# matheusfalcaopinto/triple-hybrid-rag

Measured on AMD Instinct MI355X. Metric: queries/sec (fused top-10), higher is better.
Workload: dtype f16 MFMA shortlist scan (f32 accumulate) + f64 rescoring of the f32 rows; 1 GPU; 1000000-doc / 768-d dense-only brute-force cosine top-10 (BASELINE.json configs[1]); pipeline=dense, docs=1000000, dim=768, semantic_top_k=100, fused_top_k=10, shortlist=f16, parallelism=single GPU, world_size_seen=1, rescued_queries=0

## Files before the change

triple-hybrid-rag_amd/csrc/dense.hip:

```cpp
#include <stdlib.h>

#include "dense_common.hpp"

namespace thr {

constexpr double QREG_AIM_1M = 1448.0;
constexpr int QREG_KS = 32;
struct DenseKnobs {
    bool forced_q;
    int shape;
    bool forced32;
    double aim_1m;
    int ks;
};
static const DenseKnobs& dense_knobs() {
    static const DenseKnobs knobs = [] {
        DenseKnobs K;
        const char* e = getenv("THR_DENSE_F16");
        K.forced_q = e && e[0] == 'q';
        e = getenv("THR_DENSE_MFMA");
        K.shape = (e && atoi(e) == 32) ? 32 : 16;
        e = getenv("THR_DENSE_QW");
        K.forced32 = e && atoi(e) == 32;
        e = getenv("THR_DENSE_AIM");
// ... 39 lines not shown
    p.ntiles = (n_queries + p.qtile - 1) / p.qtile;
    p.qpad = p.ntiles * p.qtile;
    const int64_t groups = (n_docs + MF_ROWS - 1) / MF_ROWS;
    p.sampled = n_docs > CAND_CAP / 2;
    const int ks_cap = p.packed ? dense_knobs().ks : 64;
    p.ksample = kprime < ks_cap ? kprime : ks_cap;
    double aim = (p.packed ? dense_knobs().aim_1m : 4096.0) * sqrt((double)n_docs / 1.0e6);
    const double aim_lo = 8.0 * kprime < 4096.0 ? 8.0 * kprime : 4096.0;
    aim = aim < aim_lo ? aim_lo : aim > 4096.0 ? 4096.0 : aim;
    int64_t target = (int64_t)((double)n_docs * (double)p.ksample / aim);
    if (target > SAMPLE_MAX) target = SAMPLE_MAX;
    if (target < 4 * (int64_t)p.ksample) target = 4 * (int64_t)p.ksample;
    int64_t sg = (target + MF_ROWS - 1) / MF_ROWS;
    if (sg > groups) sg = groups;
    p.sample_stride = sg > 0 ? groups / sg : 1;
    if (p.sample_stride < 1) p.sample_stride = 1;
    p.sample_groups = p.sampled ? sg : 0;
    p.sample_docs = p.sample_groups * MF_ROWS;
    p.groups = groups;
    p.tile_cap = p.packed ? 1 : p.qtile * (CAND_CAP / 2);
    const size_t qpad = (size_t)p.qpad;
    Arena A{(char*)ws};
    p.tau = A.take<float>(qpad);
    p.qerr = A.take<float>(qpad);
    if (kind != KIND_F16) p.qerr = nullptr;
    p.cnt = A.take<int>(qpad * (p.packed ? QREG_MAX_SEG : 1));
    p.tcnt = A.take<int>(p.ntiles);
    p.cand = A.take<Cand>(qpad * CAND_CAP);
    p.tlist = A.take<Cand>((size_t)p.ntiles * p.tile_cap);
    p.sample = A.take<float>(p.packed ? qpad * (size_t)QREG_MAX_SEG * SAMPLE_TOP : qpad * (size_t)p.sample_docs);
    p.qfrag = A.take<_Float16>(p.packed ? qpad * (size_t)dim : 0);
    p.sel_rows = A.take<int32_t>(qpad * SEL_BIG_BAND);
    p.sel_meta = A.take<int32_t>(4 * qpad);
    p.total = A.total;
    return p;
}

dim3 scan_grid(int ntiles, int64_t n_row_tiles, int waves, bool* shared_rows, int blocks_per_cu,
               int m_cap) {
    const int cus = num_cus() * blocks_per_cu;
    int64_t m_max = n_row_tiles / (8 * (int64_t)waves);
    if (m_max < 1) m_max = 1;
    if (m_max > m_cap) m_max = m_cap;
    int best_m = 1;
    double best_eff = 0.0;
    for (int m = 1; m <= (int)m_max; ++m) {
        const int64_t g = 8 * (int64_t)m * ntiles;
        const int64_t rounds = (g + cus - 1) / cus;
        const double eff = (double)g / (double)(rounds * cus);
        if (eff > best_eff + 1e-9) {
            best_eff = eff;
            best_m = m;
        }
    }
    *shared_rows = ntiles > 1;
    return dim3((unsigned)(8 * best_m * ntiles), 1u);
}

bool scan_nt(bool shared_rows) { return !shared_rows; }


template <int MODE>
static int launch_scan(const DensePlan& P, const DenseIndex& X, const DenseBatch& B, int* nseg = nullptr) {
    constexpr bool all = MODE == MODE_ALL;
    const int64_t units = all ? P.sample_groups : P.groups, stride = all ? P.sample_stride : 1;
    const float* tau = all ? nullptr : P.tau;
    float* smp = all ? P.sample : nullptr;
    const int64_t ld = all ? P.sample_docs : 0;
    if (P.packed)
        return launch_scan_f16q<MODE>(X.dim, X.docs16, P.qfrag, P.ntiles, units, stride, tau,
                                      all ? nullptr : P.cnt, all ? nullptr : P.cand, smp, B.st,
                                      nseg, X.doc_coll, B.query_coll, B.n_queries);
    const int32_t* doc_coll = all ? nullptr : X.doc_coll;
    const int32_t* query_coll = all ? nullptr : B.query_coll;
    int* tcnt = all ? nullptr : P.tcnt;
    Cand* tlist = all ? nullptr : P.tlist;
    const int tile_cap = all ? 0 : P.tile_cap;
    if (P.anydim)
        return launch_scan_anydim<MODE>(X.dim, X.docs, X.inv_norm, X.n_docs, B.queries, B.n_queries, P.ntiles,
                                        units, stride, tau, tcnt, tlist, tile_cap, smp, ld, B.st, doc_coll,
                                        query_coll);
    if (P.kind == KIND_F16)
        return launch_scan_f16<MODE>(X.dim, P.nq, X.docs, X.inv_norm, X.n_docs, B.queries, B.n_queries,
                                     P.ntiles, units, stride, tau, tcnt, tlist, tile_cap, smp, ld, B.st,
                                     doc_coll, query_coll);
    return launch_scan_mfma<MODE>(X.dim, X.docs, X.inv_norm, X.n_docs, B.queries, B.n_queries, P.ntiles,
                                  units, stride, tau, tcnt, tlist, tile_cap, smp, ld, B.st, doc_coll,
                                  query_coll);
}

static int dense_pipeline(const DensePlan& P, const DenseIndex& X, const DenseBatch& B,
                          const DensePhase& S) {
    int rc, nseg = 0, sample_nseg = 0;
    if (S.phase != PIPE_FINISH) {
        if (!P.packed) {
            hipError_t e = hipMemsetAsync(P.cnt, 0, (char*)P.cand - (char*)P.cnt, B.st);
            if (e != hipSuccess) return (int)e;
        }
        if (P.packed && (rc = launch_pack_queries(X.dim, B.queries, B.n_queries, P.qpad, P.qfrag, P.qerr, B.st)))
            return rc;
        if (P.sampled && (rc = launch_scan<MODE_ALL>(P, X, B, &sample_nseg))) return rc;
        if ((rc = launch_threshold(P, X, B, P.packed ? sample_nseg : 0))) return rc;
        if ((rc = launch_scan<MODE_FILTER>(P, X, B, &nseg))) return rc;
        if (!P.packed && (rc = launch_bucket(P, B.st))) return rc;
    } else if (P.packed) {
        if ((rc = launch_scan_f16q<MODE_FILTER, true>(X.dim, X.docs16, P.qfrag, P.ntiles, P.groups, 1,
                                                      nullptr, nullptr, nullptr, nullptr, B.st, &nseg)))
            return rc;
    }
    if ((rc = launch_band(P, X, B, S, nseg))) return rc;
    if (S.phase == PIPE_SHORTLIST) return THR_OK;
    return launch_rescore(P, X, B);
}

}

using namespace thr;

extern "C" size_t thr_dense_workspace_bytes(int64_t n_docs, int dim, int n_queries, int kprime) {
    if (n_docs <= 0 || n_queries <= 0) return 0;
    return make_plan(nullptr, n_docs, n_queries, kprime, KIND_F32, dim, false).total;
}

static int dense_args_ok(const void* docs, const void* dnorm, const void* inv_norm,
                         const void* queries, const void* a, const void* b, const void* c,
                         const void* d, const void* ws, int64_t n_docs, int n_queries, int k,
                         int kprime) {
    THR_RETURN_IF(!docs || !dnorm || !inv_norm || !queries || !a || !b || !c || !d || !ws,
                  THR_ERR_INVALID);
    THR_RETURN_IF(n_docs <= 0 || n_queries <= 0 || k <= 0 || kprime < k ||
                      kprime > THR_DENSE_MAX_K,
                  THR_ERR_INVALID);
// ... 209 lines not shown
```

triple-hybrid-rag_amd/csrc/dense_common.hpp:

```cpp
#pragma once
#include <type_traits>

#include "thr_common.hpp"

namespace thr {

constexpr int CHUNK = 256;
constexpr int MODE_ALL = 0, MODE_FILTER = 1;
constexpr int CAND_CAP = 16384;
constexpr int SAMPLE_MAX = 1 << 20;
constexpr int WBUF = 256;
constexpr int ROW_BITS = 27;
constexpr uint32_t ROW_MASK = (1u << ROW_BITS) - 1;
constexpr int ROW_BITS_F16 = 25;
constexpr int SEL_BIG_BAND = 1024;
constexpr int QREG_MAX_SEG = 1024;
constexpr int SAMPLE_TOP = 4;
constexpr int CS_BINS = 4096;

struct Cand {
    float score;
    uint32_t doc;
};

// ... 49 lines not shown
           (sizeof(Cand) * WBUF + sizeof(float4) * MF2_STAGE_F4) * H_WAVES;
}
inline int f16_pick_nq(int dim) { return f16_lds_bytes(dim, 2) <= 160 * 1024 ? 2 : 1; }

inline bool anydim_ok(int dim) {
    return dim >= THR_DENSE_ANYDIM_STEP && dim <= THR_DENSE_ANYDIM_MAX && dim % THR_DENSE_ANYDIM_STEP == 0;
}
inline int anydim_qt(int dim) { return dim <= 768 ? 64 : dim <= 1536 ? 32 : 16; }
inline size_t anydim_lds_bytes(int dim) {
    return sizeof(_Float16) * (size_t)anydim_qt(dim) * (size_t)dim + sizeof(Cand) * WBUF * H_WAVES;
}

inline bool f16_tiles_agree() {
    for (int dim : {512, 768, 1024})
        if (anydim_qt(dim) != 32 * f16_pick_nq(dim)) return false;
    return true;
}

inline double scan_eps(int dim) {
    const double u = 5.9604644775390625e-08;
    return ((double)dim + 16.0) * u;
}

constexpr int KIND_F32 = 0, KIND_F16 = 1;
struct DensePlan {
    int kind;
    bool anydim;
    bool packed;
    int nq, qtile, ntiles, qpad, row_bits, ksample, tile_cap;
    bool sampled;
    int64_t groups, sample_groups, sample_stride, sample_docs;
    float* tau;
    float* qerr;
    int* cnt;
    int* tcnt;
    Cand *cand, *tlist;
    float* sample;
    _Float16* qfrag;
    int32_t *sel_rows, *sel_meta;
    size_t total;
};
struct DenseIndex {
    const float *docs, *inv_norm;
    int64_t n_docs;
    int dim;
    const double* dnorm = nullptr;
    int64_t id_base = 0;
    const int32_t* doc_coll = nullptr;
    const _Float16* docs16 = nullptr;
    double doc_rel_err = 0.0;
};
struct DenseBatch {
    const float* queries;
    int n_queries, k, kprime;
    const int32_t* query_coll;
    hipStream_t st;
    double* out_scores = nullptr;
    int64_t* out_ids = nullptr;
    int32_t* out_counts = nullptr;
    uint32_t* out_flags = nullptr;
};
enum { PIPE_ALL = 0, PIPE_SHORTLIST = 1, PIPE_FINISH = 2 };
struct DensePhase {
    int phase = PIPE_ALL;
    float* top_lb = nullptr;
    int top_m = 0;
// ... 7 lines not shown
int qreg_shape(int dim);
int qreg_qw(int dim);
int qreg_max_queries(int dim);
dim3 scan_grid(int ntiles, int64_t n_row_tiles, int waves, bool* shared_rows, int blocks_per_cu = 1,
               int m_cap = 64);
bool scan_nt(bool shared_rows);

template <int MODE>
int launch_scan_mfma(int dim, const float* docs, const float* inv_norm, int64_t n_docs,
                     const float* queries, int n_queries, int ntiles, int64_t n_row_tiles,
                     int64_t tile_stride, const float* tau, int* tile_cnt, Cand* tile_list,
                     int tile_cap, float* sample, int64_t sample_ld, hipStream_t st,
                     const int32_t* doc_coll = nullptr, const int32_t* query_coll = nullptr);
template <int MODE>
int launch_scan_f16(int dim, int nq, const float* rows32, const float* inv_norm, int64_t n_docs,
                    const float* queries, int n_queries, int ntiles, int64_t n_row_tiles,
                    int64_t tile_stride, const float* tau, int* tile_cnt, Cand* tile_list,
                    int tile_cap, float* sample, int64_t sample_ld, hipStream_t st,
                    const int32_t* doc_coll = nullptr, const int32_t* query_coll = nullptr);
template <int MODE>
int launch_scan_anydim(int dim, const float* rows32, const float* inv_norm, int64_t n_docs,
                       const float* queries, int n_queries, int ntiles, int64_t n_row_tiles,
                       int64_t tile_stride, const float* tau, int* tile_cnt, Cand* tile_list,
                       int tile_cap, float* sample, int64_t sample_ld, hipStream_t st,
                       const int32_t* doc_coll = nullptr, const int32_t* query_coll = nullptr);
template <int MODE, bool PROF = false>
int launch_scan_f16q(int dim, const _Float16* rows16, const _Float16* qfrag, int n_qtiles,
                     int64_t n_row_tiles, int64_t tile_stride, const float* tau, int* seg_cnt,
                     Cand* cand, float* sample, hipStream_t st,
                     int* nseg_out = nullptr, const int32_t* doc_coll = nullptr,
                     const int32_t* query_coll = nullptr, int n_queries = 1 << 30,
                     unsigned long long* stamps = nullptr, int* n_blocks = nullptr);
int launch_pack_queries(int dim, const float* queries, int n_queries, int qpad, _Float16* qfrag,
                        float* qerr, hipStream_t st);
int launch_quantize_f16(const float* docs, int64_t n_docs, int dim, _Float16* docs16,
                        unsigned int* max_rel_err, hipStream_t st);
int launch_threshold(const DensePlan& P, const DenseIndex& X, const DenseBatch& B, int sample_nseg);
int launch_bucket(const DensePlan& P, hipStream_t st);
int launch_band(const DensePlan& P, const DenseIndex& X, const DenseBatch& B, const DensePhase& S, int nseg);
int launch_rescore(const DensePlan& P, const DenseIndex& X, const DenseBatch& B);
int launch_merge_scoped(const double* slab_s, const int64_t* slab_id, int n_queries, int n_slabs, int k,
                        int64_t id_base, const int32_t* query_scope, int n_scopes, double* out_scores,
                        int64_t* out_ids, int32_t* out_counts, uint32_t* out_flags, hipStream_t st);

}
```

triple-hybrid-rag_amd/csrc/dense_rescore.hip:

```cpp
#include "dense_common.hpp"

namespace thr {

constexpr int RS_STRIDE = 9;
constexpr int RR_WAVES = 2, RR_THREADS = 64 * RR_WAVES, RR_ROWS = 64;
static size_t rescore_lds_bytes(int dim) {
    return sizeof(double) * dim + sizeof(float4) * RR_WAVES * RR_ROWS * RS_STRIDE;
}
template <int U, bool TAIL = false>
__device__ __forceinline__ double rescore_pass(const f32x4* (&rp)[8], f32x4* stage, const double* q64,
                                               int nchunk, int lane, int lrow, int lch) {
    constexpr int D = U >= 2 ? 16 / U : 8;
    f32x4 nxt[D][U];
#pragma unroll
    for (int dd = 0; dd < D; ++dd)
#pragma unroll
        for (int u = 0; u < U; ++u) nxt[dd][u] = rp[u][8 * (TAIL && dd >= nchunk ? nchunk - 1 : dd)];
    double dot = 0.0;
#pragma unroll 1
    for (int ck0 = 0; ck0 < nchunk; ck0 += D) {
#pragma unroll
        for (int dd = 0; dd < D; ++dd) {
            const int ck = ck0 + dd;
            if (TAIL && ck >= nchunk) break;
// ... 84 lines not shown
        double sim = -INFINITY;
        if (dn > 0.0) sim = qn > 0.0 ? __ddiv_rn(dot, __dmul_rn(qn, dn)) : 0.0;
        s_s[p] = sim;
        s_id[p] = sim == -INFINITY ? INT64_MAX : row + id_base;
    }
    __syncthreads();
    for (int p = threadIdx.x; p < ns; p += RR_THREADS) {
        const double ms = s_s[p];
        const int64_t mi = s_id[p];
        if (mi == INT64_MAX) continue;
        int rank = 0;
        for (int i = 0; i < ns; ++i) rank += better(s_s[i], s_id[i], ms, mi) ? 1 : 0;
        o_s[rank] = ms;
        o_id[rank] = mi;
    }
    __syncthreads();

    int mine_valid = 0;
    for (int i = threadIdx.x; i < k; i += RR_THREADS) {
        const bool ok = o_s[i] > -INFINITY;
        mine_valid += ok ? 1 : 0;
        out_scores[(int64_t)q * k + i] = ok ? o_s[i] : -INFINITY;
        out_ids[(int64_t)q * k + i] = ok ? o_id[i] : -1;
    }
    if (mine_valid) atomicAdd(&n_valid, mine_valid);
    __syncthreads();
    if (threadIdx.x == 0) {
        const int valid = n_valid;
        uint32_t flag = overflow ? THR_FLAG_OVERFLOW : 0u;
        bool cert;
        if (overflow) {
            cert = false;
        } else if (floor32 == -INFINITY) {
            cert = true;
        } else {
            const float gF = __uint_as_float((uint32_t)sel_meta[4 * q + 3]);
            const bool own = valid >= k && s_qn > 0.0 && (o_s[k - 1] - (double)floor32 / s_qn) > eps;
            const bool all = gF > -INFINITY && s_qn > 0.0 &&
                             ((double)gF / s_qn - (double)floor32 / s_qn) > eps;
            cert = own || all;
        }
        out_flags[q] = flag | (cert ? THR_FLAG_CERTIFIED : 0u);
        out_counts[q] = valid;
    }
}

int launch_rescore(const DensePlan& P, const DenseIndex& X, const DenseBatch& B) {
    const bool tail = X.dim % 256 != 0, big_lds = X.dim > 1024;
    for (auto kern : {tail ? rescore_rank<THR_DENSE_MAX_K, true> : rescore_rank<THR_DENSE_MAX_K, false>,
                      tail ? rescore_rank<SEL_BIG_BAND, true> : rescore_rank<SEL_BIG_BAND, false>}) {
        int rc;
        if (big_lds) {
            rc = launch_lds(kern, dim3(B.n_queries), dim3(RR_THREADS), rescore_lds_bytes(X.dim), B.st,
                            X.docs, X.dnorm, X.dim, X.id_base, B.queries, B.k, scan_eps(X.dim),
                            X.doc_rel_err, (const float*)P.qerr, (const int32_t*)P.sel_rows,
                            (const int32_t*)P.sel_meta, B.out_scores, B.out_ids, B.out_counts, B.out_flags);
        } else {
            hipLaunchKernelGGL(kern, dim3(B.n_queries), dim3(RR_THREADS), rescore_lds_bytes(X.dim), B.st,
                               X.docs, X.dnorm, X.dim, X.id_base, B.queries, B.k, scan_eps(X.dim),
                               X.doc_rel_err, P.qerr, P.sel_rows, P.sel_meta, B.out_scores, B.out_ids,
                               B.out_counts, B.out_flags);
            rc = launch_status();
        }
        if (rc) return rc;
    }
    return THR_OK;
}
// ... 3 lines not shown
```

triple-hybrid-rag_amd/csrc/dense_scan_f16q.hip:

```cpp
#include "dense_scan_f16q.hpp"

namespace thr {

template <int MODE, bool PROF>
int launch_scan_f16q(int dim, const _Float16* rows16, const _Float16* qfrag, int n_qtiles,
                            int64_t n_row_tiles, int64_t tile_stride, const float* tau, int* seg_cnt,
                            Cand* cand, float* sample, hipStream_t st,
                            int* nseg_out, const int32_t* doc_coll,
                            const int32_t* query_coll, int n_queries,
                            unsigned long long* stamps, int* n_blocks) {
    bool shared_rows = false;
    const bool stag = qreg_staggered(dim);
    const dim3 grid = scan_grid(n_qtiles, n_row_tiles, 1, &shared_rows, (!stag && dim <= 768) ? 2 : 1, 32);
    const int shape = qreg_shape(dim);
    const int nseg = (shape == 16 ? 4 : 2) * (int)(grid.x / n_qtiles);
    if (nseg_out) *nseg_out = nseg;
    if (n_blocks) *n_blocks = (int)grid.x;
    if (PROF && !stamps) return THR_OK;
#define THR_QS_LAUNCH(DIM, SHAPE)                                                                 \
    return launch_lds(dense_scan_f16qs<DIM, MODE, SHAPE>, grid, dim3(QS_NW * 64),                 \
                      QStag<DIM>::LDS_BYTES, st, (const f32x4*)rows16, (const f32x4*)qfrag,       \
                      n_qtiles, n_row_tiles, tile_stride, tau, seg_cnt, cand, CAND_CAP / nseg,    \
                      sample, doc_coll, query_coll, n_queries);
    if (stag) {
        if (dim == 512 && shape == 32) THR_QS_LAUNCH(512, 32)
        if (dim == 512) THR_QS_LAUNCH(512, 16)
        if (shape == 32) THR_QS_LAUNCH(768, 32)
        THR_QS_LAUNCH(768, 16)
    }
#undef THR_QS_LAUNCH
#define THR_Q_LAUNCH(DIM, SHAPE)                                                                  \
    return launch_lds(dense_scan_f16q<DIM, MODE, PROF, SHAPE>, grid, dim3(Q_NW * 64),             \
                      QScan<DIM>::LDS_BYTES, st, (const f32x4*)rows16, (const f32x4*)qfrag,       \
                      n_qtiles, n_row_tiles, tile_stride, tau, seg_cnt, cand, CAND_CAP / nseg,    \
                      sample, doc_coll, query_coll, n_queries, stamps);
    switch (dim) {
        case 512: if (shape == 16) THR_Q_LAUNCH(512, 16) THR_Q_LAUNCH(512, 32)
        case 768: if (shape == 16) THR_Q_LAUNCH(768, 16) THR_Q_LAUNCH(768, 32)
        case 1024:
            if (shape == 16 && qreg_qw(dim) == 48) THR_Q_LAUNCH(1024, 48)
            if (shape == 16) THR_Q_LAUNCH(1024, 16)
            THR_Q_LAUNCH(1024, 32)
        default: return THR_ERR_UNSUPPORTED;
    }
#undef THR_Q_LAUNCH
}

int launch_pack_queries(int dim, const float* queries, int n_queries, int qpad,
                               _Float16* qfrag, float* qerr, hipStream_t st) {
    const dim3 grid((unsigned)(qpad / 32));
    const bool s16 = qreg_shape(dim) == 16;
#define THR_PACK(DIM, SHAPE) \
    hipLaunchKernelGGL((pack_queries_f16<DIM, SHAPE>), grid, dim3(256), 0, st, queries, n_queries, (f32x4*)qfrag, qerr)
    switch (dim) {
        case 512: if (s16) THR_PACK(512, 16); else THR_PACK(512, 32); break;
        case 768: if (s16) THR_PACK(768, 16); else THR_PACK(768, 32); break;
        case 1024: if (s16) THR_PACK(1024, 16); else THR_PACK(1024, 32); break;
        default: return THR_ERR_UNSUPPORTED;
    }
#undef THR_PACK
    return launch_status();
}

int launch_quantize_f16(const float* docs, int64_t n_docs, int dim, _Float16* docs16,
                        unsigned int* max_rel_err, hipStream_t st) {
    if (docs16) {
        THR_RETURN_IF(dim % 16 != 0, THR_ERR_UNSUPPORTED);
        const int64_t n_pad = (n_docs + 31) / 32 * 32;
        hipLaunchKernelGGL(quantize_f16_norm, dim3((unsigned)((n_pad + 3) / 4)), dim3(256), 0, st,
                           docs, n_docs, dim, qreg_shape(dim), docs16, max_rel_err);
        return launch_status();
    }
    hipLaunchKernelGGL(measure_f16_error, dim3((unsigned)((n_docs + 3) / 4)), dim3(256), 0, st, docs,
                       n_docs, dim, max_rel_err);
    return launch_status();
}

#define THR_INSTANTIATE(MODE, PROF)                                                                    \
    template int launch_scan_f16q<MODE, PROF>(int, const _Float16*, const _Float16*, int, int64_t, int64_t, \
                                              const float*, int*, Cand*, float*, hipStream_t, int*, \
                                              const int32_t*, const int32_t*, int, unsigned long long*, int*);
THR_INSTANTIATE(MODE_ALL, false)
THR_INSTANTIATE(MODE_FILTER, false)
THR_INSTANTIATE(MODE_FILTER, true)
#undef THR_INSTANTIATE

// ... 2 lines not shown
```

triple-hybrid-rag_amd/csrc/dense_scan_f16q.hpp:

```cpp
#pragma once
#include "dense_common.hpp"

namespace thr {

constexpr int Q_RING = 4;
constexpr int Q_NW = 4;

template <int DIM>
struct QScan {
    static constexpr int KS = DIM / 16;
    static constexpr int HS = KS / 2;
    static constexpr int HALF_BYTES = HS * 1024;
    static constexpr int PER_CU = DIM <= 768 ? 2 : 1;
    static constexpr int NB = (160 * 1024 / PER_CU) / HALF_BYTES > 4 ? 4 : (160 * 1024 / PER_CU) / HALF_BYTES;
    static constexpr int PER = HS / Q_NW;
#ifndef THR_Q_RING_1024
#define THR_Q_RING_1024 8
#endif
    static constexpr int RING = PER_CU == 1 ? THR_Q_RING_1024 : Q_RING;
#ifdef Q_PROBE_EXTRA
    static constexpr int VM_PER_PIECE = 2, LDS_BYTES = NB * HALF_BYTES + 32 * 1024;
#else
    static constexpr int VM_PER_PIECE = 1, LDS_BYTES = NB * HALF_BYTES;
#endif
    static_assert(HS % Q_NW == 0 && NB >= 3, "half tile must split evenly over the waves; >= 3 buffers");
};

template <int DIM, int SHAPE>
__global__ __launch_bounds__(256) void pack_queries_f16(const float* __restrict__ queries,
                                                        int n_queries, f32x4* __restrict__ qfrag,
                                                        float* __restrict__ qerr) {
    constexpr int KS = DIM / 16;
    const int lane = threadIdx.x & 63, wave = threadIdx.x >> 6;
    __shared__ double red[4][4][32];
    double e = 0.0, nn = 0.0, e_hi = 0.0, n_hi = 0.0;
#pragma unroll 4
    for (int s = wave; s < KS; s += 4) {
        int q, d0;
        if constexpr (SHAPE == 32) {
            q = blockIdx.x * 32 + (lane & 31);
            d0 = 16 * s + 8 * (lane >> 5);
        } else {
            q = blockIdx.x * 32 + 16 * (s / (KS / 2)) + (lane & 15);
            d0 = 32 * (s % (KS / 2)) + 8 * (lane >> 4);
        }
        f32x4 lo = {0.f, 0.f, 0.f, 0.f}, hi = lo;
        if (q < n_queries) {
            const f32x4* src = reinterpret_cast<const f32x4*>(queries + (int64_t)q * DIM + d0);
            lo = src[0];
            hi = src[1];
        }
        const f32x4 packed = pack_f16x8(lo, hi);
        qfrag[((int64_t)blockIdx.x * KS + s) * 64 + lane] = packed;
        const half8 hv = __builtin_bit_cast(half8, packed);
        double e1 = 0.0, n1 = 0.0;
#pragma unroll
        for (int j = 0; j < 8; ++j) {
            const float v = j < 4 ? lo[j] : hi[j - 4];
            const double d = (double)v - (double)(float)hv[j];
            e1 += d * d;
            n1 += (double)v * (double)v;
        }
        if (SHAPE == 32 || s < KS / 2) {
            e += e1;
            nn += n1;
        } else {
            e_hi += e1;
            n_hi += n1;
        }
    }
    if constexpr (SHAPE == 32) {
        e += __shfl_xor(e, 32, WAVE);
        nn += __shfl_xor(nn, 32, WAVE);
        if (lane < 32) {
            red[wave][0][lane] = e;
            red[wave][1][lane] = nn;
        }
    } else {
#pragma unroll
        for (int m = 16; m <= 32; m <<= 1) {
            e += __shfl_xor(e, m, WAVE);
            nn += __shfl_xor(nn, m, WAVE);
            e_hi += __shfl_xor(e_hi, m, WAVE);
            n_hi += __shfl_xor(n_hi, m, WAVE);
        }
        if (lane < 16) {
            red[wave][0][lane] = e;
            red[wave][1][lane] = nn;
            red[wave][0][16 + lane] = e_hi;
            red[wave][1][16 + lane] = n_hi;
        }
    }
    __syncthreads();
    if (threadIdx.x < 32) {
        double es = 0.0, ns = 0.0;
#pragma unroll
        for (int w = 0; w < 4; ++w) {
            es += red[w][0][threadIdx.x];
            ns += red[w][1][threadIdx.x];
        }
        const float rel = ns > 0.0 ? (float)sqrt(es / ns) : 0.f;
        qerr[blockIdx.x * 32 + threadIdx.x] = __uint_as_float(__float_as_uint(rel) + 1u);
    }
}

#define QS_RD(dst, ks) \
    asm volatile("ds_read_b128 %0, %1 offset:%2" : "=v"(dst) : "v"(abase), "n"((ks) * 1024) : "memory")
template <int S, int HS, int RING>
__device__ __forceinline__ void qs_fill(f32x4 (&a)[RING], uint32_t abase) {
    if constexpr (S < RING && S < HS) {
        QS_RD(a[S], S);
        qs_fill<S + 1, HS>(a, abase);
    }
}
template <int SHAPE>
struct QAcc;
template <>
struct QAcc<32> {
    static constexpr int NQL = 1, SEGS = 2;
    static constexpr int QW = 32, NQB = 2, NREG = 16;
    f32x16 v;
    __device__ __forceinline__ void zero() {
#pragma unroll
        for (int x = 0; x < 16; ++x) v[x] = 0.f;
    }
    template <int X> __device__ __forceinline__ float get() const { return v[X]; }
    template <int X> static __device__ __forceinline__ int row(int lane) { return (X & 3) + 8 * (X >> 2) + 4 * (lane >> 5); }
    template <int X> static constexpr int qsel() { return 0; }
    static __device__ __forceinline__ int query(int lane, int) { return lane & 31; }
    static __device__ __forceinline__ int seg(int lane) { return lane >> 5; }
};
template <>
struct QAcc<48> {
    static constexpr int NQL = 3, SEGS = 4;
    static constexpr int QW = 48, NQB = 3, NREG = 24;
// ... 70 lines not shown
            if (qc[qs] != -1 && doc_coll[row] != qc[qs]) return;
            if (slot[qs] < end[qs]) {
                const uint64_t word = (uint64_t)__float_as_uint(v) | ((uint64_t)row << 32);
                asm volatile("global_store_dwordx2 %0, %1, %2" ::"v"(slot[qs]), "v"(word), "s"(cand) : "memory");
            }
            slot[qs] += 8;
        }
    }
    template <int X>
    __device__ __forceinline__ void all(const QAcc<SHAPE>& acc, uint32_t row0, int lane) {
        if constexpr (X < QAcc<SHAPE>::NREG) {
            one<X>(acc, row0, lane);
            all<X + 1>(acc, row0, lane);
        }
    }
};

template <int SHAPE>
struct QTop {
    static constexpr int NQL = QAcc<SHAPE>::NQL;
    const int32_t* doc_coll;
    int qc[NQL];
    float t[NQL][SAMPLE_TOP];
    __device__ __forceinline__ void init() {
#pragma unroll
        for (int u = 0; u < NQL; ++u)
#pragma unroll
            for (int j = 0; j < SAMPLE_TOP; ++j) t[u][j] = -INFINITY;
    }
    template <int X>
    __device__ __forceinline__ void one(const QAcc<SHAPE>& acc, uint32_t row0, int lane) {
        constexpr int qs = QAcc<SHAPE>::template qsel<X>();
        float x = acc.template get<X>();
        x = x == x ? x : -INFINITY;
        if (doc_coll && qc[qs] != -1 && x > -INFINITY) {
            const uint32_t row = row0 + (uint32_t)QAcc<SHAPE>::template row<X>(lane);
            if (doc_coll[row] != qc[qs]) x = -INFINITY;
        }
#pragma unroll
        for (int j = 0; j < SAMPLE_TOP; ++j) {
            const float hi = fmaxf(t[qs][j], x);
            x = fminf(t[qs][j], x);
            t[qs][j] = hi;
        }
    }
    template <int X>
    __device__ __forceinline__ void all(const QAcc<SHAPE>& acc, uint32_t row0, int lane) {
        if constexpr (X < QAcc<SHAPE>::NREG) {
            one<X>(acc, row0, lane);
            all<X + 1>(acc, row0, lane);
        }
    }
    __device__ __forceinline__ void store(float* __restrict__ sample, int u, int64_t q, int nseg, int seg) const {
        float* dst = sample + (q * nseg + seg) * SAMPLE_TOP;
#pragma unroll
        for (int j = 0; j < SAMPLE_TOP; ++j) dst[j] = t[u][j];
    }
};

template <int S, int HS, int K0, int KS, int PER, int SHAPE, int HF, int RING, int NBQ, typename Issue>
__device__ __forceinline__ void qsx_steps_pe(f32x4 (&a)[RING], const f32x4 (&bq)[NBQ], QAcc<SHAPE>& acc,
                                             uint32_t abase, Issue& issue_piece, QEmit<SHAPE>& em,
                                             const QAcc<SHAPE>& prv, uint32_t row_prv, int lane) {
    if constexpr (S < HS) {
        constexpr int left = HS - S - 1 < RING - 1 ? HS - S - 1 : RING - 1;
        asm volatile("s_waitcnt lgkmcnt(%1)" : "+v"(a[S % RING]) : "n"(left) : "memory");
        qsx_mfma<S, K0, KS, SHAPE>(a[S % RING], bq, acc);
        if constexpr (S + RING < HS) QS_RD(a[S % RING], S + RING);
        constexpr int every = HS / PER;
        if constexpr (S % every == 1 && S / every < PER) issue_piece(std::integral_constant<int, S / every>{});
        constexpr int NRH = QAcc<SHAPE>::NREG / 2, j = S * NRH / HS;
        if constexpr ((S + 1) * NRH / HS > j) em.template one<NRH * HF + j>(prv, row_prv, lane);
        qsx_steps_pe<S + 1, HS, K0, KS, PER, SHAPE, HF, RING, NBQ>(a, bq, acc, abase, issue_piece, em, prv, row_prv, lane);
    }
}
#undef QS_RD

// ... 484 lines not shown
```

triple-hybrid-rag_amd/csrc/dense_select.hip:

```cpp
#include "dense_common.hpp"

namespace thr {

constexpr int BUCKET_BLOCKS = 32;
__global__ __launch_bounds__(256) void bucket_candidates(const int* __restrict__ tile_cnt,
                                                         const Cand* __restrict__ tile_list,
                                                         int tile_cap, int qtile, int row_bits,
                                                         int* __restrict__ cand_cnt,
                                                         Cand* __restrict__ cand) {
    __shared__ int count[128], base[128], fill[128];
    const uint32_t row_mask = (1u << row_bits) - 1u;
    const int tile = blockIdx.y;
    int n = tile_cnt[tile];
    n = n < tile_cap ? n : tile_cap;
    const int per = (n + gridDim.x - 1) / gridDim.x;
    const int lo = blockIdx.x * per, hi = lo + per < n ? lo + per : n;
    const Cand* list = tile_list + (int64_t)tile * tile_cap;
    if (threadIdx.x < 128) count[threadIdx.x] = fill[threadIdx.x] = 0;
    __syncthreads();
    for (int i = lo + threadIdx.x; i < hi; i += blockDim.x)
        atomicAdd(&count[list[i].doc >> row_bits], 1);
    __syncthreads();
    if (threadIdx.x < qtile && count[threadIdx.x] > 0)
        base[threadIdx.x] = atomicAdd(&cand_cnt[tile * qtile + threadIdx.x], count[threadIdx.x]);
// ... 196 lines not shown
    sweep([&](float v) { m = fmaxf(m, v); });
#pragma unroll
    for (int o = 32; o > 0; o >>= 1) m = fmaxf(m, __shfl_xor(m, o, WAVE));
    if (lane == 0) kred[wave] = m;
    if (threadIdx.x == 0) kcnt = 0;
    for (int i = threadIdx.x; i < CS_BINS; i += 256) hist[i] = 0;
    __syncthreads();
    m = fmaxf(fmaxf(kred[0], kred[1]), fmaxf(kred[2], kred[3]));
    if (m > 0.f && m < INFINITY) {
        const float thr = 0.5f * m, scale = 4095.f / (m - thr);
        int c = 0;
        sweep([&](float v) {
            if (v >= thr) {
                const int bn = (int)((v - thr) * scale);
                atomicAdd(&hist[bn > CS_BINS - 1 ? CS_BINS - 1 : bn], 1);
                ++c;
            }
        });
#pragma unroll
        for (int o = 32; o > 0; o >>= 1) c += __shfl_xor(c, o, WAVE);
        if (lane == 0 && c) atomicAdd(&kcnt, c);
        __syncthreads();
        if (kcnt >= kk) {
            coarse_find_bin(hist, kk, aux);
            if (threadIdx.x == 0) tau[q] = thr + (float)aux[0] / scale;
            return;
        }
        __syncthreads();
    }
    const uint32_t key = block_coarse_select([&](int i) { return fkey(val(i)); }, n_sample, kk, hist, aux);
    if (threadIdx.x == 0) tau[q] = coarse_value(key);
}

constexpr int KT_REG = 16;
static_assert(QREG_MAX_SEG * SAMPLE_TOP <= 256 * KT_REG, "kth_select_top holds every kept value in registers");
__global__ __launch_bounds__(256) void kth_select_top(const float* __restrict__ sample, int n_vals, int kk,
                                                      const float* __restrict__ queries, int n_queries,
                                                      int dim, float* __restrict__ tau) {
    __shared__ int hist[256];
    __shared__ int wsum[4];
    __shared__ int bc[2];
    __shared__ int flag;
    const int q = blockIdx.x, t = threadIdx.x, lane = t & 63, wave = t >> 6;
    if (query_is_void(queries, n_queries, dim, q, &flag)) {
        if (t == 0) tau[q] = INFINITY;
        return;
    }
    if (n_vals < kk) {
        if (t == 0) tau[q] = -INFINITY;
        return;
    }
    uint32_t key[KT_REG];
#pragma unroll
    for (int u = 0; u < KT_REG; ++u) {
        const int i = t + u * 256;
        key[u] = fkey(i < n_vals ? sample[(int64_t)q * n_vals + i] : -INFINITY);
    }
    uint32_t prefix = 0, mask = 0;
    int remaining = kk;
#pragma unroll 1
    for (int shift = 24; shift >= 0; shift -= 8) {
        hist[t] = 0;
        __syncthreads();
#pragma unroll
        for (int u = 0; u < KT_REG; ++u)
            if (t + u * 256 < n_vals && (key[u] & mask) == prefix) atomicAdd(&hist[(key[u] >> shift) & 255], 1);
        __syncthreads();
        const int mine = hist[255 - t];
        int incl = mine;
#pragma unroll
        for (int o = 1; o < 64; o <<= 1) {
            const int v = __shfl_up(incl, o, WAVE);
            if (lane >= o) incl += v;
        }
        if (lane == 63) wsum[wave] = incl;
        __syncthreads();
        for (int x = 0; x < wave; ++x) incl += wsum[x];
        if (incl - mine < remaining && remaining <= incl) {
            bc[0] = 255 - t;
            bc[1] = incl - mine;
        }
        __syncthreads();
        remaining -= bc[1];
        prefix |= (uint32_t)bc[0] << shift;
        mask |= 255u << shift;
    }
    if (t == 0) tau[q] = fkey_inv(prefix);
}

constexpr int SEL_THREADS = 256;
constexpr int SEL_REG = 16;
constexpr int SEL_FLAT = 8192;
static size_t band_lds_bytes(int dim) { return sizeof(float) * dim + sizeof(int) * CS_BINS; }
constexpr int CAPB = SEL_BIG_BAND;
template <bool TOPM>
__global__ __launch_bounds__(SEL_THREADS, 4) void select_band(
    int dim, const float* __restrict__ queries, const float* __restrict__ tau,
    const int* __restrict__ cand_cnt, const Cand* __restrict__ cand,
    const int* __restrict__ tile_cnt, int tile_cap, int qtile, int k, int kprime, double eps32,
    double doc_relerr, const float* __restrict__ qerr, int nseg, int seg_cap,
    const int32_t* __restrict__ doc_coll, const int32_t* __restrict__ query_coll,
    int32_t* __restrict__ sel_rows, int32_t* __restrict__ sel_meta,
    const float* __restrict__ gfloor, const float* __restrict__ lb_all, int n_shards, int lb_m,
    float* __restrict__ top_lb, int top_m) {
    extern __shared__ float4 lds_sel[];
    __shared__ int aux[8];
    __shared__ int bc[4];
    __shared__ int32_t s_id[CAPB];
    __shared__ int n_sel;
    __shared__ double wsum[4];
    float* lds_qv = reinterpret_cast<float*>(lds_sel);
    int* hist = reinterpret_cast<int*>(lds_sel + dim / 4);

    const int q = blockIdx.x;
    const int lane = threadIdx.x & 63, wave = threadIdx.x >> 6;
    const double eq = qerr ? (double)qerr[q] : 0.0;
    const double eps = eps32 + doc_relerr * (1.0 + eq) + eq;
    const Cand* c = cand + (int64_t)q * CAND_CAP;
    const Cand* my_ptr = c + threadIdx.x;
    int my_n, my_c[4] = {0, 0, 0, 0};
    bool overflow, flat = true;
    int n;
    __shared__ unsigned short src_off[SEL_FLAT];
    if (nseg == 0) {
        const int cnt = cand_cnt[q];
        overflow = cnt > CAND_CAP || tile_cnt[q / qtile] > tile_cap;
        n = cnt < CAND_CAP ? cnt : CAND_CAP;
        my_n = n > (int)threadIdx.x ? (n - (int)threadIdx.x + SEL_THREADS - 1) / SEL_THREADS : 0;
    } else {
        __shared__ int wtot[4];
        bool over = false;
        int tot = 0;
#pragma unroll
        for (int x = 0; x < 4; ++x) {
            const int sg = (int)threadIdx.x + x * SEL_THREADS;
            int sc = sg < nseg ? cand_cnt[(int64_t)q * nseg + sg] : 0;
            over |= sc > seg_cap;
// ... 31 lines not shown
        int sg = threadIdx.x;
#pragma unroll
        for (int x = 0; x < 3; ++x)
            if (u >= my_c[x]) {
                u -= my_c[x];
                sg += SEL_THREADS;
            } else {
                break;
            }
        return c[(int64_t)sg * seg_cap + u];
    };

    const int qc = query_coll ? query_coll[q] : -1;
    auto load_cand = [&](int u) -> Cand {
        Cand e = cand_at(u);
        if (qc != -1 && doc_coll[e.doc] != qc) e.score = -INFINITY;
        return e;
    };
    Cand mine[SEL_REG];
#pragma unroll
    for (int u = 0; u < SEL_REG; ++u) mine[u] = u < my_n ? load_cand(u) : Cand{-INFINITY, 0u};
    if (qc != -1) {
        __shared__ int n_pass;
        if (threadIdx.x == 0) n_pass = 0;
        __syncthreads();
        int mine_ok = 0;
#pragma unroll
        for (int u = 0; u < SEL_REG; ++u) mine_ok += (u < my_n && mine[u].score > -INFINITY) ? 1 : 0;
        for (int u = SEL_REG; u < my_n; ++u) mine_ok += load_cand(u).score > -INFINITY ? 1 : 0;
        if (mine_ok) atomicAdd(&n_pass, mine_ok);
        __syncthreads();
        n = n_pass;
    }
    for (int i = threadIdx.x; i < dim / 4; i += SEL_THREADS)
        lds_sel[i] = reinterpret_cast<const float4*>(queries + (int64_t)q * dim)[i];
    if (threadIdx.x == 0) n_sel = 0;
    __syncthreads();

    {
        double part = 0.0;
        for (int i = threadIdx.x; i < dim; i += SEL_THREADS) part += (double)lds_qv[i] * (double)lds_qv[i];
        for (int o = 32; o > 0; o >>= 1) part += __shfl_xor(part, o, WAVE);
        if (lane == 0) wsum[wave] = part;
        __syncthreads();
    }
    const double qn_hi = sqrt(wsum[0] + wsum[1] + wsum[2] + wsum[3]) * (1.0 + 1e-6);

    float gF = -INFINITY;
    if (!TOPM) {
        if (gfloor) {
            gF = gfloor[q];
        } else if (lb_all && n_shards * lb_m >= k) {
            __shared__ float s_gF;
            float* fv = reinterpret_cast<float*>(hist);
            const int nv = n_shards * lb_m, nv4 = (nv + 3) & ~3;
            for (int i = threadIdx.x; i < nv4; i += SEL_THREADS)
                fv[i] = i < nv ? lb_all[((int64_t)(i / lb_m) * gridDim.x + q) * lb_m + i % lb_m] : -INFINITY;
            if (threadIdx.x == 0) s_gF = -INFINITY;
            __syncthreads();
            const f32x4* fv4 = reinterpret_cast<const f32x4*>(fv);
            for (int i = threadIdx.x; i < nv; i += SEL_THREADS) {
                const float v = fv[i];
                if (!(v > -INFINITY)) continue;
                int rank = 0;
#pragma unroll 4
                for (int j = 0; j < nv4; j += 4) {
                    const f32x4 w = fv4[j >> 2];
                    rank += (w.x > v || (w.x == v && j < i)) ? 1 : 0;
                    rank += (w.y > v || (w.y == v && j + 1 < i)) ? 1 : 0;
                    rank += (w.z > v || (w.z == v && j + 2 < i)) ? 1 : 0;
                    rank += (w.w > v || (w.w == v && j + 3 < i)) ? 1 : 0;
                }
                if (rank == k - 1) s_gF = v;
            }
            __syncthreads();
            gF = s_gF;
            __syncthreads();
        }
    }
// ... 175 lines not shown
    for (int i = threadIdx.x; i < ns; i += SEL_THREADS) sel_rows[(int64_t)q * CAPB + i] = s_id[i];
    if (threadIdx.x == 0) {
        sel_meta[4 * q + 0] = ns;
        sel_meta[4 * q + 1] = (int32_t)__float_as_uint(floor32);
        sel_meta[4 * q + 2] = overflow ? 1 : 0;
        sel_meta[4 * q + 3] = (int32_t)__float_as_uint(gF);
    }
}

__global__ __launch_bounds__(256) void dense_floor_kernel(const float* __restrict__ lb, int n_shards,
                                                          int n_queries, int m, int k,
                                                          float* __restrict__ gfloor) {
    extern __shared__ float fl_v[];
    const int q = blockIdx.x, n = n_shards * m;
    for (int i = threadIdx.x; i < n; i += blockDim.x)
        fl_v[i] = lb[((int64_t)(i / m) * n_queries + q) * m + i % m];
    if (threadIdx.x == 0) gfloor[q] = -INFINITY;
    __syncthreads();
    if (n < k) return;
    for (int i = threadIdx.x; i < n; i += blockDim.x) {
        const float v = fl_v[i];
        if (!(v > -INFINITY)) continue;
        int rank = 0;
        for (int j = 0; j < n; ++j) {
            const float w = fl_v[j];
            rank += (w > v || (w == v && j < i)) ? 1 : 0;
        }
        if (rank == k - 1) gfloor[q] = v;
    }
}

int launch_threshold(const DensePlan& P, const DenseIndex& X, const DenseBatch& B, int sample_nseg) {
    if (P.sampled && sample_nseg > 0) {
        hipLaunchKernelGGL(kth_select_top, dim3(P.qpad), dim3(256), 0, B.st, (const float*)P.sample,
                           sample_nseg * SAMPLE_TOP, P.ksample, B.queries, B.n_queries, X.dim, P.tau);
        return launch_status();
    }
    hipLaunchKernelGGL(kth_select, dim3(P.qpad), dim3(256), 0, B.st,
                       P.sampled ? (const float*)P.sample : nullptr, P.sample_docs, (int)P.sample_docs,
                       P.ksample, B.queries, B.n_queries, X.dim, P.tau, P.packed ? nullptr : P.qerr,
                       X.doc_coll, B.query_coll, MF_ROWS, P.sampled ? P.sample_stride : (int64_t)1,
                       X.n_docs);
    return launch_status();
}

int launch_bucket(const DensePlan& P, hipStream_t st) {
    hipLaunchKernelGGL(bucket_candidates, dim3(BUCKET_BLOCKS, P.ntiles), dim3(256), 0, st, P.tcnt,
                       P.tlist, P.tile_cap, P.qtile, P.row_bits, P.cnt, P.cand);
    return launch_status();
}

int launch_band(const DensePlan& P, const DenseIndex& X, const DenseBatch& B, const DensePhase& S,
                int nseg) {
    const bool topm = S.phase == PIPE_SHORTLIST;
    hipLaunchKernelGGL(topm ? select_band<true> : select_band<false>, dim3(B.n_queries),
                       dim3(SEL_THREADS), band_lds_bytes(X.dim), B.st, X.dim, B.queries, P.tau, P.cnt,
                       P.cand, P.tcnt, P.tile_cap, P.qtile, B.k, B.kprime, scan_eps(X.dim),
                       X.doc_rel_err, P.qerr, nseg, nseg ? CAND_CAP / nseg : 0, X.doc_coll,
                       B.query_coll, P.sel_rows, P.sel_meta, S.gfloor, S.lb_all, S.n_shards,
                       topm ? 0 : S.top_m, S.top_lb, topm ? S.top_m : 0);
    return launch_status();
}

}

using namespace thr;

extern "C" int thr_dense_floor(const float* top_lb, int n_shards, int n_queries, int m, int k,
                               float* gfloor, thr_stream_t stream) {
    clear_status();
    THR_RETURN_IF(!top_lb || !gfloor || n_shards <= 0 || n_queries <= 0 || m <= 0 || k <= 0, THR_ERR_INVALID);
    THR_RETURN_IF((int64_t)n_shards * m > 8192, THR_ERR_CAPACITY);
    hipLaunchKernelGGL(dense_floor_kernel, dim3(n_queries), dim3(256), sizeof(float) * n_shards * m,
                       (hipStream_t)stream, top_lb, n_shards, n_queries, m, k, gfloor);
    return launch_status();
}
```

Measured before the change: 756,100 queries/s.

## Precompute query norms and void flags in pack kernel; wave-level kth select

The query-packing kernel now also writes each query's f64 norm bound and an all-zero flag. The select_band kernel can then skip reloading the query and re-reducing its norm, and the threshold kernel no longer rescans the query to detect void queries. kth_select_top is rewritten to process one query per wave with a bitwise ballot radix select, replacing the block-wide shared-memory histogram passes. The sampled top-4 insertion uses fmed3 instead of a max/min chain, and the NaN guard moves from the scan to a NaN check on the norm in the rescore certification. The change adds workspace buffers and shifts NaN handling semantics.

Result: no change. 760,600 queries/s (median of 6 runs) (+0.6%).

```diff
diff --git a/triple-hybrid-rag_amd/csrc/dense.hip b/triple-hybrid-rag_amd/csrc/dense.hip
--- a/triple-hybrid-rag_amd/csrc/dense.hip
+++ b/triple-hybrid-rag_amd/csrc/dense.hip
@@ -95,6 +95,8 @@
     p.qfrag = A.take<_Float16>(p.packed ? qpad * (size_t)dim : 0);
     p.sel_rows = A.take<int32_t>(qpad * SEL_BIG_BAND);
     p.sel_meta = A.take<int32_t>(4 * qpad);
+    p.qn_hi = p.packed ? A.take<double>(qpad) : nullptr;
+    p.qvoid = p.packed ? A.take<int>(qpad) : nullptr;
     p.total = A.total;
     return p;
 }
@@ -160,7 +162,7 @@
             hipError_t e = hipMemsetAsync(P.cnt, 0, (char*)P.cand - (char*)P.cnt, B.st);
             if (e != hipSuccess) return (int)e;
         }
-        if (P.packed && (rc = launch_pack_queries(X.dim, B.queries, B.n_queries, P.qpad, P.qfrag, P.qerr, B.st)))
+        if (P.packed && (rc = launch_pack_queries(X.dim, B.queries, B.n_queries, P.qpad, P.qfrag, P.qerr, P.qn_hi, P.qvoid, B.st)))
             return rc;
         if (P.sampled && (rc = launch_scan<MODE_ALL>(P, X, B, &sample_nseg))) return rc;
         if ((rc = launch_threshold(P, X, B, P.packed ? sample_nseg : 0))) return rc;
diff --git a/triple-hybrid-rag_amd/csrc/dense_common.hpp b/triple-hybrid-rag_amd/csrc/dense_common.hpp
--- a/triple-hybrid-rag_amd/csrc/dense_common.hpp
+++ b/triple-hybrid-rag_amd/csrc/dense_common.hpp
@@ -105,6 +105,8 @@
     int64_t groups, sample_groups, sample_stride, sample_docs;
     float* tau;
     float* qerr;
+    double* qn_hi;
+    int* qvoid;
     int* cnt;
     int* tcnt;
     Cand *cand, *tlist;
@@ -178,7 +180,7 @@
                      const int32_t* query_coll = nullptr, int n_queries = 1 << 30,
                      unsigned long long* stamps = nullptr, int* n_blocks = nullptr);
 int launch_pack_queries(int dim, const float* queries, int n_queries, int qpad, _Float16* qfrag,
-                        float* qerr, hipStream_t st);
+                        float* qerr, double* qn_hi, int* qvoid, hipStream_t st);
 int launch_quantize_f16(const float* docs, int64_t n_docs, int dim, _Float16* docs16,
                         unsigned int* max_rel_err, hipStream_t st);
 int launch_threshold(const DensePlan& P, const DenseIndex& X, const DenseBatch& B, int sample_nseg);
diff --git a/triple-hybrid-rag_amd/csrc/dense_rescore.hip b/triple-hybrid-rag_amd/csrc/dense_rescore.hip
--- a/triple-hybrid-rag_amd/csrc/dense_rescore.hip
+++ b/triple-hybrid-rag_amd/csrc/dense_rescore.hip
@@ -140,7 +140,7 @@
         if (overflow) {
             cert = false;
         } else if (floor32 == -INFINITY) {
-            cert = true;
+            cert = s_qn == s_qn;
         } else {
             const float gF = __uint_as_float((uint32_t)sel_meta[4 * q + 3]);
             const bool own = valid >= k && s_qn > 0.0 && (o_s[k - 1] - (double)floor32 / s_qn) > eps;
diff --git a/triple-hybrid-rag_amd/csrc/dense_scan_f16q.hip b/triple-hybrid-rag_amd/csrc/dense_scan_f16q.hip
--- a/triple-hybrid-rag_amd/csrc/dense_scan_f16q.hip
+++ b/triple-hybrid-rag_amd/csrc/dense_scan_f16q.hip
@@ -47,11 +47,11 @@
 }
 
 int launch_pack_queries(int dim, const float* queries, int n_queries, int qpad,
-                               _Float16* qfrag, float* qerr, hipStream_t st) {
+                               _Float16* qfrag, float* qerr, double* qn_hi, int* qvoid, hipStream_t st) {
     const dim3 grid((unsigned)(qpad / 32));
     const bool s16 = qreg_shape(dim) == 16;
 #define THR_PACK(DIM, SHAPE) \
-    hipLaunchKernelGGL((pack_queries_f16<DIM, SHAPE>), grid, dim3(256), 0, st, queries, n_queries, (f32x4*)qfrag, qerr)
+    hipLaunchKernelGGL((pack_queries_f16<DIM, SHAPE>), grid, dim3(256), 0, st, queries, n_queries, (f32x4*)qfrag, qerr, qn_hi, qvoid)
     switch (dim) {
         case 512: if (s16) THR_PACK(512, 16); else THR_PACK(512, 32); break;
         case 768: if (s16) THR_PACK(768, 16); else THR_PACK(768, 32); break;
diff --git a/triple-hybrid-rag_amd/csrc/dense_scan_f16q.hpp b/triple-hybrid-rag_amd/csrc/dense_scan_f16q.hpp
--- a/triple-hybrid-rag_amd/csrc/dense_scan_f16q.hpp
+++ b/triple-hybrid-rag_amd/csrc/dense_scan_f16q.hpp
@@ -29,11 +29,14 @@
 template <int DIM, int SHAPE>
 __global__ __launch_bounds__(256) void pack_queries_f16(const float* __restrict__ queries,
                                                         int n_queries, f32x4* __restrict__ qfrag,
-                                                        float* __restrict__ qerr) {
+                                                        float* __restrict__ qerr,
+                                                        double* __restrict__ qn_hi, int* __restrict__ qvoid) {
     constexpr int KS = DIM / 16;
     const int lane = threadIdx.x & 63, wave = threadIdx.x >> 6;
     __shared__ double red[4][4][32];
+    __shared__ int nzs[4][32];
     double e = 0.0, nn = 0.0, e_hi = 0.0, n_hi = 0.0;
+    int nz = 0, nz_hi = 0;
 #pragma unroll 4
     for (int s = wave; s < KS; s += 4) {
         int q, d0;
@@ -54,27 +57,33 @@
         qfrag[((int64_t)blockIdx.x * KS + s) * 64 + lane] = packed;
         const half8 hv = __builtin_bit_cast(half8, packed);
         double e1 = 0.0, n1 = 0.0;
+        int z1 = 0;
 #pragma unroll
         for (int j = 0; j < 8; ++j) {
             const float v = j < 4 ? lo[j] : hi[j - 4];
             const double d = (double)v - (double)(float)hv[j];
             e1 += d * d;
             n1 += (double)v * (double)v;
+            z1 |= v != 0.f ? 1 : 0;
         }
         if (SHAPE == 32 || s < KS / 2) {
             e += e1;
             nn += n1;
+            nz |= z1;
         } else {
             e_hi += e1;
             n_hi += n1;
+            nz_hi |= z1;
         }
     }
     if constexpr (SHAPE == 32) {
         e += __shfl_xor(e, 32, WAVE);
         nn += __shfl_xor(nn, 32, WAVE);
+        nz |= __shfl_xor(nz, 32, WAVE);
         if (lane < 32) {
             red[wave][0][lane] = e;
             red[wave][1][lane] = nn;
+            nzs[wave][lane] = nz;
         }
     } else {
 #pragma unroll
@@ -83,12 +92,16 @@
             nn += __shfl_xor(nn, m, WAVE);
             e_hi += __shfl_xor(e_hi, m, WAVE);
             n_hi += __shfl_xor(n_hi, m, WAVE);
+            nz |= __shfl_xor(nz, m, WAVE);
+            nz_hi |= __shfl_xor(nz_hi, m, WAVE);
         }
         if (lane < 16) {
             red[wave][0][lane] = e;
             red[wave][1][lane] = nn;
             red[wave][0][16 + lane] = e_hi;
             red[wave][1][16 + lane] = n_hi;
+            nzs[wave][lane] = nz;
+            nzs[wave][16 + lane] = nz_hi;
         }
     }
     __syncthreads();
@@ -101,6 +114,9 @@
         }
         const float rel = ns > 0.0 ? (float)sqrt(es / ns) : 0.f;
         qerr[blockIdx.x * 32 + threadIdx.x] = __uint_as_float(__float_as_uint(rel) + 1u);
+        qn_hi[blockIdx.x * 32 + threadIdx.x] = sqrt(ns) * (1.0 + 1e-6);
+        qvoid[blockIdx.x * 32 + threadIdx.x] =
+            (nzs[0][threadIdx.x] | nzs[1][threadIdx.x] | nzs[2][threadIdx.x] | nzs[3][threadIdx.x]) ? 0 : 1;
     }
 }
 
@@ -237,17 +253,14 @@
     __device__ __forceinline__ void one(const QAcc<SHAPE>& acc, uint32_t row0, int lane) {
         constexpr int qs = QAcc<SHAPE>::template qsel<X>();
         float x = acc.template get<X>();
-        x = x == x ? x : -INFINITY;
         if (doc_coll && qc[qs] != -1 && x > -INFINITY) {
             const uint32_t row = row0 + (uint32_t)QAcc<SHAPE>::template row<X>(lane);
             if (doc_coll[row] != qc[qs]) x = -INFINITY;
         }
-#pragma unroll
-        for (int j = 0; j < SAMPLE_TOP; ++j) {
-            const float hi = fmaxf(t[qs][j], x);
-            x = fminf(t[qs][j], x);
-            t[qs][j] = hi;
-        }
+        float* s = t[qs];
+#pragma unroll
+        for (int j = SAMPLE_TOP - 1; j > 0; --j) s[j] = __builtin_amdgcn_fmed3f(s[j - 1], s[j], x);
+        s[0] = fmaxf(s[0], x);
     }
     template <int X>
     __device__ __forceinline__ void all(const QAcc<SHAPE>& acc, uint32_t row0, int lane) {
diff --git a/triple-hybrid-rag_amd/csrc/dense_select.hip b/triple-hybrid-rag_amd/csrc/dense_select.hip
--- a/triple-hybrid-rag_amd/csrc/dense_select.hip
+++ b/triple-hybrid-rag_amd/csrc/dense_select.hip
@@ -252,60 +252,41 @@
     if (threadIdx.x == 0) tau[q] = coarse_value(key);
 }
 
-constexpr int KT_REG = 16;
-static_assert(QREG_MAX_SEG * SAMPLE_TOP <= 256 * KT_REG, "kth_select_top holds every kept value in registers");
-__global__ __launch_bounds__(256) void kth_select_top(const float* __restrict__ sample, int n_vals, int kk,
-                                                      const float* __restrict__ queries, int n_queries,
-                                                      int dim, float* __restrict__ tau) {
-    __shared__ int hist[256];
-    __shared__ int wsum[4];
-    __shared__ int bc[2];
-    __shared__ int flag;
-    const int q = blockIdx.x, t = threadIdx.x, lane = t & 63, wave = t >> 6;
-    if (query_is_void(queries, n_queries, dim, q, &flag)) {
-        if (t == 0) tau[q] = INFINITY;
+constexpr int KT_WAVES = 4;
+static_assert(QREG_MAX_SEG * SAMPLE_TOP <= 64 * WAVE, "kth_select_top holds every kept value in registers");
+template <int PER>
+__global__ __launch_bounds__(64 * KT_WAVES) void kth_select_top(const float* __restrict__ sample, int n_vals, int kk,
+                                                                const int* __restrict__ qvoid, int qpad,
+                                                                float* __restrict__ tau) {
+    const int lane = threadIdx.x & 63;
+    const int q = __builtin_amdgcn_readfirstlane((int)(blockIdx.x * KT_WAVES + (threadIdx.x >> 6)));
+    if (q >= qpad) return;
+    if (qvoid[q]) {
+        if (lane == 0) tau[q] = INFINITY;
         return;
     }
     if (n_vals < kk) {
-        if (t == 0) tau[q] = -INFINITY;
+        if (lane == 0) tau[q] = -INFINITY;
         return;
     }
-    uint32_t key[KT_REG];
-#pragma unroll
-    for (int u = 0; u < KT_REG; ++u) {
-        const int i = t + u * 256;
-        key[u] = fkey(i < n_vals ? sample[(int64_t)q * n_vals + i] : -INFINITY);
-    }
-    uint32_t prefix = 0, mask = 0;
+    uint32_t key[PER];
+#pragma unroll
+    for (int u = 0; u < PER; ++u) {
+        const int i = lane + u * WAVE;
+        key[u] = i < n_vals ? fkey(sample[(int64_t)q * n_vals + i]) : 0u;
+    }
+    uint32_t prefix = 0;
     int remaining = kk;
 #pragma unroll 1
-    for (int shift = 24; shift >= 0; shift -= 8) {
-        hist[t] = 0;
-        __syncthreads();
-#pragma unroll
-        for (int u = 0; u < KT_REG; ++u)
-            if (t + u * 256 < n_vals && (key[u] & mask) == prefix) atomicAdd(&hist[(key[u] >> shift) & 255], 1);
-        __syncthreads();
-        const int mine = hist[255 - t];
-        int incl = mine;
-#pragma unroll
-        for (int o = 1; o < 64; o <<= 1) {
-            const int v = __shfl_up(incl, o, WAVE);
-            if (lane >= o) incl += v;
-        }
-        if (lane == 63) wsum[wave] = incl;
-        __syncthreads();
-        for (int x = 0; x < wave; ++x) incl += wsum[x];
-        if (incl - mine < remaining && remaining <= incl) {
-            bc[0] = 255 - t;
-            bc[1] = incl - mine;
-        }
-        __syncthreads();
-        remaining -= bc[1];
-        prefix |= (uint32_t)bc[0] << shift;
-        mask |= 255u << shift;
-    }
-    if (t == 0) tau[q] = fkey_inv(prefix);
+    for (int b = 31; b >= 0; --b) {
+        const uint32_t want = (prefix >> b) | 1u;
+        int cnt = 0;
+#pragma unroll
+        for (int u = 0; u < PER; ++u) cnt += __popcll(__ballot((key[u] >> b) == want));
+        if (cnt >= remaining) prefix |= 1u << b;
+        else remaining -= cnt;
+    }
+    if (lane == 0) tau[q] = fkey_inv(prefix);
 }
 
 constexpr int SEL_THREADS = 256;
@@ -322,7 +303,7 @@
     const int32_t* __restrict__ doc_coll, const int32_t* __restrict__ query_coll,
     int32_t* __restrict__ sel_rows, int32_t* __restrict__ sel_meta,
     const float* __restrict__ gfloor, const float* __restrict__ lb_all, int n_shards, int lb_m,
-    float* __restrict__ top_lb, int top_m) {
+    float* __restrict__ top_lb, int top_m, const double* __restrict__ qn_hi_in) {
     extern __shared__ float4 lds_sel[];
     __shared__ int aux[8];
     __shared__ int bc[4];
@@ -420,19 +401,22 @@
         __syncthreads();
         n = n_pass;
     }
-    for (int i = threadIdx.x; i < dim / 4; i += SEL_THREADS)
-        lds_sel[i] = reinterpret_cast<const float4*>(queries + (int64_t)q * dim)[i];
+    double qn_hi;
     if (threadIdx.x == 0) n_sel = 0;
-    __syncthreads();
-
-    {
+    if (qn_hi_in) {
+        qn_hi = qn_hi_in[q];
+        __syncthreads();
+    } else {
+        for (int i = threadIdx.x; i < dim / 4; i += SEL_THREADS)
+            lds_sel[i] = reinterpret_cast<const float4*>(queries + (int64_t)q * dim)[i];
+        __syncthreads();
         double part = 0.0;
         for (int i = threadIdx.x; i < dim; i += SEL_THREADS) part += (double)lds_qv[i] * (double)lds_qv[i];
         for (int o = 32; o > 0; o >>= 1) part += __shfl_xor(part, o, WAVE);
         if (lane == 0) wsum[wave] = part;
         __syncthreads();
-    }
-    const double qn_hi = sqrt(wsum[0] + wsum[1] + wsum[2] + wsum[3]) * (1.0 + 1e-6);
+        qn_hi = sqrt(wsum[0] + wsum[1] + wsum[2] + wsum[3]) * (1.0 + 1e-6);
+    }
 
     float gF = -INFINITY;
     if (!TOPM) {
@@ -674,8 +658,12 @@
 
 int launch_threshold(const DensePlan& P, const DenseIndex& X, const DenseBatch& B, int sample_nseg) {
     if (P.sampled && sample_nseg > 0) {
-        hipLaunchKernelGGL(kth_select_top, dim3(P.qpad), dim3(256), 0, B.st, (const float*)P.sample,
-                           sample_nseg * SAMPLE_TOP, P.ksample, B.queries, B.n_queries, X.dim, P.tau);
+        const int n_vals = sample_nseg * SAMPLE_TOP;
+        THR_RETURN_IF(n_vals > 64 * WAVE, THR_ERR_CAPACITY);
+        const dim3 grid((unsigned)((P.qpad + KT_WAVES - 1) / KT_WAVES));
+        auto kern = n_vals <= 8 * WAVE ? kth_select_top<8> : n_vals <= 16 * WAVE ? kth_select_top<16> : kth_select_top<64>;
+        hipLaunchKernelGGL(kern, grid, dim3(64 * KT_WAVES), 0, B.st, (const float*)P.sample, n_vals, P.ksample,
+                           (const int*)P.qvoid, P.qpad, P.tau);
         return launch_status();
     }
     hipLaunchKernelGGL(kth_select, dim3(P.qpad), dim3(256), 0, B.st,
@@ -700,7 +688,7 @@
                        P.cand, P.tcnt, P.tile_cap, P.qtile, B.k, B.kprime, scan_eps(X.dim),
                        X.doc_rel_err, P.qerr, nseg, nseg ? CAND_CAP / nseg : 0, X.doc_coll,
                        B.query_coll, P.sel_rows, P.sel_meta, S.gfloor, S.lb_all, S.n_shards,
-                       topm ? 0 : S.top_m, S.top_lb, topm ? S.top_m : 0);
+                       topm ? 0 : S.top_m, S.top_lb, topm ? S.top_m : 0, (const double*)P.qn_hi);
     return launch_status();
 }
 
```
